# davrempe/humor

Hardware: AMD Instinct MI355X
Metric: fitting closure evaluations/s (stage-3 objective fwd+bwd), batch=32 seq=60 per GPU (higher is better)
Workload: dtype f32

## Files before the change

humor_amd/csrc/rollout.hip:

```cpp
#include <string.h>

#include <algorithm>
#include <list>
#include <unordered_map>
#include <vector>

#include "rollout_persist.h"
#include "rot_math.h"

namespace ha {

constexpr int D_IN = 339, D_STATE = 348, ZD = 48, NJT = 22, NBODY = 21;
template <int ROTW>
struct RawLayout {
  static constexpr int ROOT = 6, RVEL = 6 + ROTW, BODY = 9 + ROTW, JNT = 9 + 22 * ROTW, JVEL = JNT + 66, CONT = JVEL + 66, D = CONT + 9;
};
static_assert(RawLayout<3>::D == 216 && RawLayout<6>::D == 282 && RawLayout<9>::D == 348, "decoder output widths of the three representations");
constexpr int D_INP = 340;
constexpr int SLICE = 64;
constexpr int MAXL = 8;

typedef float f32x16 __attribute__((ext_vector_type(16)));
typedef float vf4 __attribute__((ext_vector_type(4)));

// ... 222 lines not shown
        const vf4 g4 = *reinterpret_cast<const vf4*>(T.gamma + cbase + 32 * hi + 4 * j);
        const vf4 b4 = *reinterpret_cast<const vf4*>(T.beta + cbase + 32 * hi + 4 * j);
        gam[4 * j] = g4.x; gam[4 * j + 1] = g4.y; gam[4 * j + 2] = g4.z; gam[4 * j + 3] = g4.w;
        bet[4 * j] = b4.x; bet[4 * j + 1] = b4.y; bet[4 * j + 2] = b4.z; bet[4 * j + 3] = b4.w;
      }
    }
    float a[32], h[32];
    if (!is_main) load_frag_n<true>(T.skip, 1, L.RT, T.skip_dim, rt, cbase, lane, a);
    else {
      load_frag_n<LEAN>(T.src, T.nsplit_src, L.RT, T.Csrc, rt, cbase, lane, a);
      if (!LEAN && T.mode == 3) load_frag_n(T.hsrc, T.nsplit_h, L.RT, T.Ch, rt, cbase, lane, h);
    }
    HA_TS(1, false);
    HA_TS(2, true);
    if (!LEAN && is_main && T.mode == 1 && T.hsum_dst && tile == 0 && T.nsplit_src > 1) {
      const int c0 = cbase + 32 * hi;
      float* hd = T.hsum_dst + (size_t)rt * T.Csrc * 32 + (size_t)(c0 >> 2) * 128 + (size_t)(lane & 31) * 4;
#pragma unroll
      for (int jq = 0; jq < 8; ++jq)
        if (c0 + 4 * jq < T.Csrc) *reinterpret_cast<vf4*>(hd + (size_t)jq * 128) = vf4{a[4 * jq], a[4 * jq + 1], a[4 * jq + 2], a[4 * jq + 3]};
    }
    if (has_gn) {
      const float inv_n = T.inv_group;
      if (T.mode == 1) {
        if (T.group == SLICE) gn_apply<1>(1, gam, bet, inv_n, a, a);
        else gn_apply<2>(1, gam, bet, inv_n, a, a);
      } else {
        if (T.group == SLICE) gn_apply<1>(3, gam, bet, inv_n, h, a);
        else gn_apply<2>(3, gam, bet, inv_n, h, a);
      }
    }
    HA_TS(3, false);
#pragma unroll
    for (int kp = 0; kp < 32; ++kp) acc = __builtin_amdgcn_mfma_f32_32x32x2f32(a[kp], bw[kp], acc, 0, 0, 0);
  }
#pragma unroll
  for (int i = 0; i < 16; ++i) smem[(wave * 16 + i) * 64 + lane] = acc[i];
  HA_TS(4, true);
  __syncthreads();
  HA_TS(5, false);
  if (threadIdx.x < 256) {
    const int row = threadIdx.x & 31, cq = threadIdx.x >> 5;
    const int reg = (row & 3) + 4 * (row >> 3), half = (row >> 2) & 1;
    vf4 o = {0.f, 0.f, 0.f, 0.f};
#pragma unroll
    for (int w = 0; w < NWT; ++w) o += *reinterpret_cast<const vf4*>(smem + (w * 16 + reg) * 64 + half * 32 + cq * 4);
    const int n = tile * 32 + cq * 4;
    if (ks == 0 && T.bias) {
#pragma unroll
      for (int e = 0; e < 4; ++e)
        if (n + e < T.Nout) o[e] += T.bias[n + e];
    }
    float* dst = T.dst + ((size_t)ks * L.RT + rt) * T.Nout_pad * 32 + (size_t)(n >> 2) * 128 + row * 4;
    *reinterpret_cast<vf4*>(dst) = o;
  }
  HA_TS(6, true);
  HA_TS(7, false);
}

struct FinishLaunch {
  LayerTask t[1];
  float* dst[1];
  int nblk[1];
  int ntasks, RT;
};

__global__ __launch_bounds__(256) void gn_finish_kernel(FinishLaunch F) {
  extern __shared__ __attribute__((aligned(16))) float smem[];
  float (*s_red)[32][8] = reinterpret_cast<float (*)[32][8]>(smem);
  const int b = blockIdx.x, ti = 0;
  const LayerTask& T = F.t[0];
  const int row = threadIdx.x & 31, oct = threadIdx.x >> 5;
  const int slice = b % T.main_slices, rt = b / T.main_slices;
  const int c0 = slice * SLICE + oct * 8;
  const vf4 g0 = *reinterpret_cast<const vf4*>(T.gamma + c0), g1 = *reinterpret_cast<const vf4*>(T.gamma + c0 + 4);
  const vf4 e0 = *reinterpret_cast<const vf4*>(T.beta + c0), e1 = *reinterpret_cast<const vf4*>(T.beta + c0 + 4);
  auto load8 = [&](const float* base, int ns, int C, float (&v)[8]) {
    const size_t stride = (size_t)F.RT * C * 32;
    const float* p = base + (size_t)rt * C * 32 + (size_t)(c0 >> 2) * 128 + (size_t)row * 4;
    vf4 t0[MAXSPLIT], t1[MAXSPLIT];
#pragma unroll
    for (int k = 0; k < MAXSPLIT; ++k) {
      t0[k] = vf4{0.f, 0.f, 0.f, 0.f};
      t1[k] = t0[k];
      if (k < ns) { t0[k] = *reinterpret_cast<const vf4*>(p + k * stride); t1[k] = *reinterpret_cast<const vf4*>(p + k * stride + 128); }
    }
    vf4 a0 = t0[0], a1 = t1[0];
#pragma unroll
    for (int k = 1; k < MAXSPLIT; ++k) { a0 += t0[k]; a1 += t1[k]; }
    v[0] = a0.x; v[1] = a0.y; v[2] = a0.z; v[3] = a0.w; v[4] = a1.x; v[5] = a1.y; v[6] = a1.z; v[7] = a1.w;
  };
  float x[8], da[8];
  if (T.mode == 1) load8(T.src, T.nsplit_src, T.Csrc, x);
  else { load8(T.src, T.nsplit_src, T.Csrc, da); load8(T.hsrc, T.nsplit_h, T.Ch, x); }
  const float gam[8] = {g0.x, g0.y, g0.z, g0.w, g1.x, g1.y, g1.z, g1.w};
  const float bet[8] = {e0.x, e0.y, e0.z, e0.w, e1.x, e1.y, e1.z, e1.w};
  const int per = T.group == SLICE ? 8 : 4, o0 = T.group == SLICE ? 0 : (oct & 4);
  const float inv_n = 1.0f / (float)T.group;
  auto row_sum = [&](int pass, float v) {
    s_red[pass][row][oct] = v;
    __syncthreads();
    float t = 0.f;
    for (int k = 0; k < per; ++k) t += s_red[pass][row][o0 + k];
    return t;
  };
  float p1 = 0.f;
#pragma unroll
  for (int i = 0; i < 8; ++i) p1 += x[i];
  const float mu = row_sum(0, p1) * inv_n;
  float p2 = 0.f;
#pragma unroll
  for (int i = 0; i < 8; ++i) { const float d = x[i] - mu; p2 = fmaf(d, d, p2); }
  const float rstd = rsqrtf(row_sum(1, p2) * inv_n + 1e-5f);
  float out[8];
  if (T.mode == 1) {
#pragma unroll
    for (int i = 0; i < 8; ++i) out[i] = fmaxf((x[i] - mu) * rstd * gam[i] + bet[i], 0.f);
  } else {
    float xh[8], dxh[8], m1 = 0.f, m2 = 0.f;
#pragma unroll
    for (int i = 0; i < 8; ++i) {
      xh[i] = (x[i] - mu) * rstd;
      const float y = xh[i] * gam[i] + bet[i];
      dxh[i] = (y > 0.f ? da[i] : 0.f) * gam[i];
      m1 += dxh[i];
      m2 = fmaf(dxh[i], xh[i], m2);
    }
    m1 = row_sum(2, m1) * inv_n;
    m2 = row_sum(3, m2) * inv_n;
#pragma unroll
    for (int i = 0; i < 8; ++i) out[i] = rstd * (dxh[i] - m1 - xh[i] * m2);
  }
  float* d = F.dst[ti] + (size_t)rt * (T.main_slices * SLICE) * 32 + (size_t)(c0 >> 2) * 128 + (size_t)row * 4;
  *reinterpret_cast<vf4*>(d) = vf4{out[0], out[1], out[2], out[3]};
  *reinterpret_cast<vf4*>(d + 128) = vf4{out[4], out[5], out[6], out[7]};
}


struct GemmTask {
  const float* Wp; const float* bias;
  int ntiles, nslices, Nout;
  const float* src; int Csrc;
  int nrt;
  int epi;
  float slope;
  const float* gamma; const float* beta; int group;
  const float* hsrc; int Ch;
  float* dst_h; float* dst_a; int Cdst;
  int nrg, nwork, per_xcd;
};

constexpr int GEMM_LDS_WAVE = 2 * 8 * 132;

template <int RM, int KS = 1>
__global__ __launch_bounds__(256) void prior_gemm_kernel(GemmTask T) {
  extern __shared__ __attribute__((aligned(16))) float smem[];
  const int wave = threadIdx.x >> 6, lane = threadIdx.x & 63;
  const int w = (int)(blockIdx.x & 7) * T.per_xcd + (int)(blockIdx.x >> 3);
  if ((int)(blockIdx.x >> 3) >= T.per_xcd || w >= T.nwork) return;
  const int cb = w / T.nrg, rg = w % T.nrg;
  const int kpart = KS == 1 ? 0 : wave % KS;
  const int ct0 = KS == 1 ? (cb * 4 + wave) * 2 : (cb * (4 / KS) + wave / KS) * 2;
  const bool tile_ok = ct0 < T.ntiles;
  if (KS == 1 && !tile_ok) return;
  const int ct1 = ct0 + 1 < T.ntiles ? ct0 + 1 : ct0;
  int rt[RM];
#pragma unroll
  for (int m = 0; m < RM; ++m) rt[m] = rg * RM + m < T.nrt ? rg * RM + m : T.nrt - 1;

  f32x16 acc[RM][2];
#pragma unroll
  for (int m = 0; m < RM; ++m)
#pragma unroll
    for (int c = 0; c < 2; ++c)
#pragma unroll
      for (int i = 0; i < 16; ++i) acc[m][c][i] = 0.f;

  const float* wp0 = T.Wp + (size_t)ct0 * T.nslices * 2048 + lane * 4;
  const float* wp1 = T.Wp + (size_t)ct1 * T.nslices * 2048 + lane * 4;
  auto load_b = [&](int slice, float (&b0)[32], float (&b1)[32]) {
#pragma unroll
    for (int j = 0; j < 8; ++j) {
      const vf4 u = *reinterpret_cast<const vf4*>(wp0 + (size_t)slice * 2048 + j * 256);
      const vf4 v = *reinterpret_cast<const vf4*>(wp1 + (size_t)slice * 2048 + j * 256);
      b0[4 * j] = u.x; b0[4 * j + 1] = u.y; b0[4 * j + 2] = u.z; b0[4 * j + 3] = u.w;
      b1[4 * j] = v.x; b1[4 * j + 1] = v.y; b1[4 * j + 2] = v.z; b1[4 * j + 3] = v.w;
    }
  };
  auto load_a = [&](int slice, float (&a)[RM][32]) {
#pragma unroll
    for (int m = 0; m < RM; ++m)
      load_frag<1>(T.src + (size_t)rt[m] * T.Csrc * 32 + (size_t)(slice * 16 + 8 * (lane >> 5)) * 128 + (size_t)(lane & 31) * 4, 0, 8, a[m]);
  };
  auto mma = [&](const float (&a)[RM][32], const float (&b0)[32], const float (&b1)[32]) {
#pragma unroll
    for (int kp = 0; kp < 32; ++kp)
#pragma unroll
      for (int m = 0; m < RM; ++m) {
        acc[m][0] = __builtin_amdgcn_mfma_f32_32x32x2f32(a[m][kp], b0[kp], acc[m][0], 0, 0, 0);
        acc[m][1] = __builtin_amdgcn_mfma_f32_32x32x2f32(a[m][kp], b1[kp], acc[m][1], 0, 0, 0);
      }
  };
  const int nfull_all = T.Csrc / SLICE < T.nslices ? T.Csrc / SLICE : T.nslices;
  const int per_part = (nfull_all + KS - 1) / KS;
  const int sbeg = KS == 1 ? 0 : (kpart * per_part < nfull_all ? kpart * per_part : nfull_all);
  const int nfull = KS == 1 ? nfull_all : ((sbeg + per_part) < nfull_all ? (sbeg + per_part) : nfull_all);
  if (nfull > sbeg && (KS == 1 || tile_ok)) {
    float aA[RM][32], bA0[32], bA1[32], aB[RM][32], bB0[32], bB1[32];
    load_b(sbeg, bA0, bA1);
    load_a(sbeg, aA);
    for (int slice = sbeg; slice < nfull; slice += 2) {
      const int s1 = slice + 1 < nfull ? slice + 1 : slice;
      load_b(s1, bB0, bB1);
      load_a(s1, aB);
      HA_SCHED_FENCE();
      mma(aA, bA0, bA1);
      HA_SCHED_FENCE();
      if (slice + 1 < nfull) {
        const int s2 = slice + 2 < nfull ? slice + 2 : slice + 1;
        load_b(s2, bA0, bA1);
        load_a(s2, aA);
        HA_SCHED_FENCE();
        mma(aB, bB0, bB1);
        HA_SCHED_FENCE();
      }
    }
  }
  if (nfull_all < T.nslices && kpart == KS - 1 && (KS == 1 || tile_ok)) {
    float a[RM][32], b0[32], b1[32];
    load_b(nfull_all, b0, b1);
#pragma unroll
    for (int m = 0; m < RM; ++m) load_frag_n<true>(T.src, 1, 0, T.Csrc, rt[m], nfull_all * SLICE, lane, a[m]);
    mma(a, b0, b1);
  }

  float* sl = smem + wave * GEMM_LDS_WAVE;
  const int row = lane & 31, hh = lane >> 5;
  const int ct = hh ? ct0 + 1 : ct0;
  const bool ct_ok = ct < T.ntiles;
  float gam[32], bet[32];
  if ((T.epi == 1 || T.epi == 3) && ct_ok) {
#pragma unroll
    for (int j = 0; j < 8; ++j) {
      const vf4 g4 = *reinterpret_cast<const vf4*>(T.gamma + ct * 32 + 4 * j);
      const vf4 b4 = *reinterpret_cast<const vf4*>(T.beta + ct * 32 + 4 * j);
      gam[4 * j] = g4.x; gam[4 * j + 1] = g4.y; gam[4 * j + 2] = g4.z; gam[4 * j + 3] = g4.w;
      bet[4 * j] = b4.x; bet[4 * j + 1] = b4.y; bet[4 * j + 2] = b4.z; bet[4 * j + 3] = b4.w;
    }
  } else {
#pragma unroll
    for (int k = 0; k < 32; ++k) { gam[k] = 1.f; bet[k] = 0.f; }
  }
#pragma unroll
  for (int m = 0; m < RM; ++m) {
#pragma unroll
    for (int c = 0; c < 2; ++c)
#pragma unroll
      for (int i = 0; i < 16; ++i) {
        const int r = (i & 3) + 8 * (i >> 2) + 4 * hh, col = lane & 31;
        sl[(c * 8 + (col >> 2)) * 132 + r * 4 + (col & 3)] = acc[m][c][i];
      }
    if (KS == 1) {
      __builtin_amdgcn_fence(__ATOMIC_RELEASE, "wavefront");
      __builtin_amdgcn_wave_barrier();
      __builtin_amdgcn_fence(__ATOMIC_ACQUIRE, "wavefront");
    } else {
      __syncthreads();
    }
    float v[32];
#pragma unroll
    for (int j = 0; j < 8; ++j) {
      vf4 q = *reinterpret_cast<const vf4*>(sl + (hh * 8 + j) * 132 + row * 4);
      if (KS > 1) {
#pragma unroll
        for (int pk = 1; pk < KS; ++pk) q += *reinterpret_cast<const vf4*>(sl + pk * GEMM_LDS_WAVE + (hh * 8 + j) * 132 + row * 4);
      }
      v[4 * j] = q.x; v[4 * j + 1] = q.y; v[4 * j + 2] = q.z; v[4 * j + 3] = q.w;
    }
    if (KS == 1) {
      __builtin_amdgcn_fence(__ATOMIC_RELEASE, "wavefront");
      __builtin_amdgcn_wave_barrier();
      __builtin_amdgcn_fence(__ATOMIC_ACQUIRE, "wavefront");
    } else {
      __syncthreads();
      if (kpart != 0) continue;
    }
    const bool live = ct_ok && rg * RM + m < T.nrt;
    if (T.bias && ct_ok) {
#pragma unroll
      for (int j = 0; j < 8; ++j) {
        const vf4 b4 = *reinterpret_cast<const vf4*>(T.bias + ct * 32 + 4 * j);
        v[4 * j] += b4.x; v[4 * j + 1] += b4.y; v[4 * j + 2] += b4.z; v[4 * j + 3] += b4.w;
      }
    }
    const size_t o = (size_t)rt[m] * T.Cdst * 32 + (size_t)(ct * 8) * 128 + (size_t)row * 4;
    auto store32 = [&](float* base, const float (&x)[32]) {
#pragma unroll
      for (int j = 0; j < 8; ++j) *reinterpret_cast<vf4*>(base + o + (size_t)j * 128) = vf4{x[4 * j], x[4 * j + 1], x[4 * j + 2], x[4 * j + 3]};
    };
    if (T.epi <= 1 && live) store32(T.dst_h, v);
    if (T.epi == 4) {
#pragma unroll
      for (int k = 0; k < 32; ++k) v[k] = v[k] > 0.f ? v[k] : v[k] * T.slope;
      if (live) store32(T.dst_a, v);
    } else if (T.epi == 5) {
      const float* hp = T.hsrc + (size_t)rt[m] * T.Ch * 32 + (size_t)((ct_ok ? ct : ct0) * 8) * 128 + (size_t)row * 4;
#pragma unroll
      for (int j = 0; j < 8; ++j) {
        const vf4 q = *reinterpret_cast<const vf4*>(hp + (size_t)j * 128);
        v[4 * j] *= q.x > 0.f ? 1.f : T.slope; v[4 * j + 1] *= q.y > 0.f ? 1.f : T.slope;
        v[4 * j + 2] *= q.z > 0.f ? 1.f : T.slope; v[4 * j + 3] *= q.w > 0.f ? 1.f : T.slope;
      }
      if (live) store32(T.dst_a, v);
    } else if (T.epi == 1) {
      const float inv_n = 1.0f / (float)T.group;
      if (T.group == SLICE) gn_apply<1>(1, gam, bet, inv_n, v, v);
      else gn_apply<2>(1, gam, bet, inv_n, v, v);
      if (live) store32(T.dst_a, v);
    } else if (T.epi == 3) {
      float h[32];
      const float* hp = T.hsrc + (size_t)rt[m] * T.Ch * 32 + (size_t)((ct_ok ? ct : ct0) * 8) * 128 + (size_t)row * 4;
#pragma unroll
      for (int j = 0; j < 8; ++j) {
        const vf4 q = *reinterpret_cast<const vf4*>(hp + (size_t)j * 128);
        h[4 * j] = q.x; h[4 * j + 1] = q.y; h[4 * j + 2] = q.z; h[4 * j + 3] = q.w;
      }
      const float inv_n = 1.0f / (float)T.group;
      if (T.group == SLICE) gn_apply<1>(3, gam, bet, inv_n, h, v);
      else gn_apply<2>(3, gam, bet, inv_n, h, v);
      if (live) store32(T.dst_a, v);
    }
  }
}

struct GlueParams {
  int B, S, t, RT;
  const float* xT;
  float* xT_next;
  const float* dec_out; int dec_nsplit; int dec_pad;
  const float* pri_out; int pri_nsplit; int pri_pad;
  const float* Gs;
  float* Gs_next;
  const float* t2j;
  float* world;
  float* prior_mu; float* prior_var;
  const float* g_world;
  const float* g_prior_mu; const float* g_prior_var;
  float* g_dec_out;
  float* g_pri_out;
  const float* gx_dir_in;
  float* gx_dir_out;
  const float* gxp_pri; int gxp_pri_nsplit; int gxp_pri_pad;
  const float* gxp_dec; int gxp_dec_nsplit; int gxp_dec_pad;
  float* carry;
  const float* dz_src[MAXL]; int dz_nsplit[MAXL]; int dz_pad[MAXL]; int dz_off[MAXL]; int dz_n;
  float* g_z;
  float* g_past0;
};

__device__ __forceinline__ float tsum(const float* base, int nsplit, int RT, int C, int rt, int c, int row) {
  return base ? slab_sum(base, nsplit, RT, C, rt, c, row) : 0.f;
}

struct PredState {
  float pj[3], jv[3];
  float dB[9], Bin[9], pB[9];
  float ptrans[3], ptvel[3], prvel[3], dR[9], Rin[9], pR[9];
  float raw_aa_b[9], raw_aa_r[9];
};

template <int ROTW>
__device__ __forceinline__ void delta_rot(const float* raw, float R[9]) {
  if constexpr (ROTW == 3) rodrigues(raw, R);
  else if constexpr (ROTW == 6) rot6d_to_rotmat(raw, R);
  else rot9d_to_rotmat(raw, R);
}
template <int ROTW>
__device__ __forceinline__ void delta_rot_bwd(const float* raw, const float gR[9], float* graw) {
  if constexpr (ROTW == 3) rodrigues_bwd(raw, gR, graw);
  else if constexpr (ROTW == 6) rot6d_to_rotmat_bwd(raw, gR, graw);
  else rot9d_to_rotmat_bwd(raw, gR, graw);
}

constexpr int S_X = 0, S_RAW = 352, S_GXN = 704, S_GW = 1056, S_TOTAL = 1408;
constexpr int S_SH = 1408, S_RED = 1424, S_TOTAL_BWD = 1456;

template <int NQ, int NT = 64>
__device__ __forceinline__ void stage_slabs(float* dst, const float* base, int nsplit, int RT, int C, int nch, int rt, int rr,
                                            int lane, bool accumulate) {
  vf4 t[MAXSPLIT][NQ];
#pragma unroll
  for (int sidx = 0; sidx < MAXSPLIT; ++sidx)
#pragma unroll
    for (int i = 0; i < NQ; ++i) t[sidx][i] = vf4{0.f, 0.f, 0.f, 0.f};
  if (base) {
    const size_t stride = (size_t)RT * C * 32;
    const float* p0 = base + (size_t)rt * C * 32 + (size_t)rr * 4;
#pragma unroll
    for (int sidx = 0; sidx < MAXSPLIT; ++sidx)
      if (sidx < nsplit) {
#pragma unroll
        for (int i = 0; i < NQ; ++i) {
          const int q = lane + NT * i;
          if (4 * q < nch) t[sidx][i] = *reinterpret_cast<const vf4*>(p0 + (size_t)sidx * stride + (size_t)q * 128);
        }
      }
  }
#pragma unroll
  for (int i = 0; i < NQ; ++i) {
    vf4 v = {0.f, 0.f, 0.f, 0.f};
#pragma unroll
    for (int sidx = 0; sidx < MAXSPLIT; ++sidx) v += t[sidx][i];
    const int q = lane + NT * i;
#pragma unroll
    for (int e = 0; e < 4; ++e) {
      const int c = 4 * q + e;
      if (c < nch) dst[c] = accumulate ? dst[c] + v[e] : v[e];
    }
  }
}

template <int ROTW, bool DELTA>
__device__ __forceinline__ void predict_joints(const float* sX, const float* sRAW, int j, PredState& s) {
  using RL = RawLayout<ROTW>;
#pragma unroll
  for (int c = 0; c < 3; ++c) {
    s.pj[c] = sRAW[RL::JNT + 3 * j + c] + (DELTA ? sX[207 + 3 * j + c] : 0.f);
    s.jv[c] = sRAW[RL::JVEL + 3 * j + c] + (DELTA ? sX[273 + 3 * j + c] : 0.f);
  }
}
template <int ROTW, bool DELTA>
__device__ __forceinline__ void predict_body(const float* sX, const float* sRAW, int bidx, PredState& s) {
  using RL = RawLayout<ROTW>;
#pragma unroll
  for (int c = 0; c < ROTW; ++c) s.raw_aa_b[c] = sRAW[RL::BODY + ROTW * bidx + c];
  delta_rot<ROTW>(s.raw_aa_b, s.dB);
  if constexpr (DELTA) {
#pragma unroll
// ... 698 lines not shown
      HA_REQUIRE(d->gn_gamma[i] && d->gn_beta[i], "%s: layer %d GroupNorm affine missing", name, i);
      HA_REQUIRE(cin % 16 == 0 && (cin / 16 == 64 || cin / 16 == 32), "%s: hidden width %d needs GroupNorm groups of 32 or 64 channels", name, cin);
    }
    int rc = pack_layer(out[i], d->w[i], d->b[i], d->gn_gamma[i], d->gn_beta[i], cin, d->skip_dim, d->out_dims[i], gn);
    if (rc != HA_OK) return rc;
    cin = d->out_dims[i];
  }
  return HA_OK;
}

struct StashLayout {
  int RT = 0;
  int nsf_pri[MAXL], nsf_dec[MAXL], nsb_dec[MAXL];
  size_t zT = 0, t2j = 0, per_step = 0, steps = 0;
  size_t xT = 0;
  size_t off_G = 0;
  size_t off_dec[MAXL];
  size_t off_hsum[MAXL];
  size_t pri_h[MAXL];
  size_t pri_act[2];
  size_t gx_pri = 0;
  size_t smp_pri[MAXL];
  size_t gx_dir[2], carry = 0, g_dec_out = 0, g_pri_out = 0;
  size_t bwd_dec[MAXL];
  size_t fin[1] = {0};
  bool finish = false;
  bool hsum = false;
  bool single = false;
  bool pipe = false;
  size_t persist_ws = 0;
  size_t off_gn[3] = {0, 0, 0}, off_gl = 0;
  size_t off_ht[3] = {0, 0, 0};
  size_t dz_part = 0;
  int rd_f(int i) const { return single ? 1 : nsf_dec[i]; }
  size_t total = 0;
};

static bool one_launch_fits(int rows) { return g_layer_finish != 2 && (rows <= 32 || (rows <= 256 && g_rollout_pipe != 0)); }

static void make_layout(const ha_humor_net* net, int B, int S, Path path, StashLayout& L) {
  L.RT = ceil_div(B, 32);
  const size_t RT = L.RT;
  for (int i = 0; i < net->n_pri; ++i) L.nsf_pri[i] = ceil_div(net->pri[i].nslices_f, SPB);
  for (int i = 0; i < net->n_dec; ++i) { L.nsf_dec[i] = ceil_div(net->dec[i].nslices_f, SPB); L.nsb_dec[i] = ceil_div(net->dec[i].nslices_b, SPB); }
  L.finish = (L.RT >= 2 && g_layer_finish != 0) || g_layer_finish == 2;
  L.single = path != Path::chain;
  L.pipe = L.single && B > 32;
  L.hsum = !L.finish && !L.single;
  size_t o = 0;
  auto take = [&](size_t n) { size_t r = o; o += (n + 63) / 64 * 64; return r; };
  L.zT = take((size_t)S * RT * ZD * 32);
  L.t2j = take(RT * 32 * 3);
  L.xT = take((size_t)(S + 1) * RT * D_INP * 32);
  size_t p = 0;
  auto ptake = [&](size_t n) { size_t r = p; p += (n + 63) / 64 * 64; return r; };
  L.off_G = ptake(RT * 32 * 12);
  for (int i = 0; i < net->n_dec; ++i) L.off_dec[i] = ptake((size_t)L.rd_f(i) * RT * net->dec[i].Nout_pad * 32);
  for (int i = 0; i + 1 < net->n_dec; ++i) L.off_hsum[i] = L.hsum ? ptake(RT * net->dec[i].Nout_pad * 32) : 0;
  if (L.single) {
    for (int i = 0; i < 3; ++i) L.off_gn[i] = ptake(RT * 16 * 32 * 2);
    L.off_gl = ptake(RT * 32 * 32);
    for (int i = 0; i < 3; ++i) L.off_ht[i] = ptake(RT * 32 * (size_t)net->dec[i].Nout);
  }
  L.per_step = p;
  L.steps = take(p * (size_t)(S + 1));
  size_t widest = 0;
  for (int i = 0; i < net->n_pri; ++i) {
    L.pri_h[i] = take((size_t)S * RT * net->pri[i].Nout_pad * 32);
    if ((size_t)net->pri[i].Nout_pad > widest) widest = net->pri[i].Nout_pad;
    if ((size_t)net->pri[i].Nin_pad > widest) widest = net->pri[i].Nin_pad;
    L.smp_pri[i] = take((size_t)L.nsf_pri[i] * RT * net->pri[i].Nout_pad * 32);
  }
  L.pri_act[0] = take((size_t)S * RT * widest * 32);
  L.pri_act[1] = take((size_t)S * RT * widest * 32);
  L.gx_pri = take((size_t)S * RT * net->pri[0].Nin_pad * 32);
  L.gx_dir[0] = take(RT * D_INP * 32);
  L.gx_dir[1] = take(RT * D_INP * 32);
  L.carry = take(RT * 32 * 16);
  L.g_dec_out = take(RT * net->dec[net->n_dec - 1].Nout_pad * 32);
  L.g_pri_out = take((size_t)S * RT * net->pri[net->n_pri - 1].Nout_pad * 32);
  for (int i = 0; i < net->n_dec; ++i) L.bwd_dec[i] = take((size_t)L.nsb_dec[i] * RT * net->dec[i].Nin_pad * 32);
  if (L.finish)
    L.fin[0] = take(RT * 1280 * 32);
  if (L.single) {
    L.persist_ws = take(L.pipe ? pipe_ws_floats() : persist_ws_floats());
    L.dz_part = take((size_t)S * (L.pipe ? pipe_dz_slots() : persist_dz_slots()) * RT * 32 * ZD);
  }
  L.total = o;
}

static void fwd_task(LayerTask& T, const PackedLayer& L, const float* src, int nsplit_src, const float* skip, float* dst, int nsplit_dst) {
  memset(&T, 0, sizeof(T));
  T.Wp = L.Wf; T.bias = L.bias;
  T.ntiles = L.ntiles_f; T.nslices = L.nslices_f; T.main_slices = L.main_slices; T.Nout = L.Nout; T.Nout_pad = L.Nout_pad;
  T.src = src; T.nsplit_src = nsplit_src; T.Csrc = (L.Cin + 3) & ~3;
  T.skip = skip; T.skip_dim = L.skip;
  T.mode = L.group ? 1 : 0;
  T.gamma = L.gamma; T.beta = L.beta; T.group = L.group ? L.group : 64;
  T.inv_group = 1.0f / (float)T.group;
  T.dst = dst;
  T.spb = SPB; T.nsplit_dst = nsplit_dst;
  T.nblocks = L.ntiles_f * nsplit_dst;
}

static void bwd_task(LayerTask& T, const PackedLayer& L, const float* dsrc, int nsplit_d, int dC, const PackedLayer* Lnext_gn,
                     const float* hsrc, int nsplit_h, float* dst, int nsplit_dst) {
  memset(&T, 0, sizeof(T));
  T.Wp = L.Wb; T.bias = nullptr;
  T.ntiles = L.ntiles_b; T.nslices = L.nslices_b; T.main_slices = L.nslices_b; T.Nout = L.Cin + L.skip; T.Nout_pad = L.Nin_pad;
  T.src = dsrc; T.nsplit_src = nsplit_d; T.Csrc = dC;
  T.mode = Lnext_gn ? 3 : 0;
  if (Lnext_gn) { T.gamma = Lnext_gn->gamma; T.beta = Lnext_gn->beta; T.group = Lnext_gn->group; }
  else T.group = 64;
  T.inv_group = 1.0f / (float)T.group;
  T.hsrc = hsrc; T.nsplit_h = nsplit_h; T.Ch = L.Nout_pad;
  T.dst = dst;
  T.spb = SPB; T.nsplit_dst = nsplit_dst;
  T.nblocks = L.ntiles_b * nsplit_dst;
}

static int launch_layers(LayerLaunch& LL, const StashLayout& L, float* stash, hipStream_t st) {
  if (L.finish) {
    FinishLaunch F;
    memset(&F, 0, sizeof(F));
    F.RT = LL.RT;
    int fb = 0;
    for (int i = 0; i < LL.ntasks; ++i) {
      LayerTask& T = LL.t[i];
      if (T.mode == 0) continue;
      const int k = F.ntasks++;
      F.t[k] = T;
      F.dst[k] = stash + L.fin[i];
      F.nblk[k] = LL.RT * T.main_slices;
      fb += F.nblk[k];
      T.src = F.dst[k]; T.nsplit_src = 1; T.Csrc = T.main_slices * SLICE; T.mode = 0;
      T.hsrc = nullptr; T.nsplit_h = 0;
    }
    if (fb) {
      HA_LAUNCH(gn_finish_kernel, dim3(fb), dim3(256), 4 * 32 * 8 * sizeof(float), st, F);
      HA_LAUNCH_CHECK();
    }
  }
  LayerTask& T0 = LL.t[0];
  const dim3 grid(T0.ntiles, T0.nsplit_dst, LL.RT);
  T0.nblocks *= LL.RT;
  const bool lean = L.finish && T0.mode == 0 && T0.nsplit_src <= 1;
  if (lean) HA_LAUNCH((mlp_layer_kernel<4, true>), grid, dim3(256), 4 * 1024 * sizeof(float), st, LL);
  else HA_LAUNCH((mlp_layer_kernel<4, false>), grid, dim3(256), 4 * 1024 * sizeof(float), st, LL);
  HA_LAUNCH_CHECK();
  return HA_OK;
}


static int launch_prior_gemm(GemmTask& T, hipStream_t st) {
  HA_REQUIRE((T.epi != 1 && T.epi != 3) || (T.ntiles % 2 == 0 && (T.group == 32 || T.group == 64)), "prior GEMM: GroupNorm epilogue needs whole 64-column pairs");
  int ncb = ceil_div(T.ntiles, 8);
  const int rm = g_gemm_rm == 1 || g_gemm_rm == 2 ? g_gemm_rm : ((T.nrt / 2) * ncb >= 2 * 256 ? 2 : 1);
  const int ks = ((g_gemm_ks == 2 || g_gemm_ks == 3) && rm == 1 && T.nslices >= 4 && (g_gemm_ks == 3 || ncb * T.nrt * 4 <= 512)) ? 2 : 1;
  if (ks == 2) ncb = ceil_div(T.ntiles, 4);
  T.nrg = ceil_div(T.nrt, rm);
  T.nwork = ncb * T.nrg;
  T.per_xcd = ceil_div(T.nwork, 8);
  const dim3 grid(T.per_xcd * 8), block(256);
  const size_t lds = 4 * GEMM_LDS_WAVE * sizeof(float);
  if (rm == 2) HA_LAUNCH(prior_gemm_kernel<2>, grid, block, lds, st, T);
  else if (ks == 2) HA_LAUNCH((prior_gemm_kernel<1, 2>), grid, block, lds, st, T);
  else HA_LAUNCH(prior_gemm_kernel<1>, grid, block, lds, st, T);
  HA_LAUNCH_CHECK();
  return HA_OK;
}

static int prior_forward_batched(const ha_humor_net* net, const StashLayout& L, float* stash, int S, hipStream_t st) {
  const int np = net->n_pri;
  for (int l = 0; l < np; ++l) {
    const PackedLayer& P = net->pri[l];
    GemmTask T;
    memset(&T, 0, sizeof(T));
    T.Wp = P.Wf; T.bias = P.bias;
    T.ntiles = P.ntiles_f; T.nslices = P.nslices_f; T.Nout = P.Nout;
    T.src = l == 0 ? stash + L.xT : stash + L.pri_act[(l - 1) & 1];
    T.Csrc = l == 0 ? D_INP : net->pri[l - 1].Nout_pad;
    T.nrt = S * L.RT;
    T.dst_h = stash + L.pri_h[l]; T.Cdst = P.Nout_pad;
    if (l + 1 < np) {
      const PackedLayer& N = net->pri[l + 1];
      T.epi = 1; T.gamma = N.gamma; T.beta = N.beta; T.group = N.group;
      T.dst_a = stash + L.pri_act[l & 1];
    }
    int rc = launch_prior_gemm(T, st);
    if (rc != HA_OK) return rc;
  }
  return HA_OK;
}

static int prior_backward_batched(const ha_humor_net* net, const StashLayout& L, float* stash, int S, hipStream_t st) {
  const int np = net->n_pri;
  for (int l = np - 1; l >= 0; --l) {
    const PackedLayer& P = net->pri[l];
    GemmTask T;
    memset(&T, 0, sizeof(T));
    T.Wp = P.Wb; T.bias = nullptr;
    T.ntiles = P.ntiles_b; T.nslices = P.nslices_b; T.Nout = P.Cin + P.skip;
    T.src = l == np - 1 ? stash + L.g_pri_out : stash + L.pri_act[(l + 1) & 1];
    T.Csrc = P.Nout_pad;
    T.nrt = S * L.RT;
    T.Cdst = P.Nin_pad;
    if (l > 0) {
      T.epi = 3; T.gamma = P.gamma; T.beta = P.beta; T.group = P.group;
      T.hsrc = stash + L.pri_h[l - 1]; T.Ch = net->pri[l - 1].Nout_pad;
      T.dst_a = stash + L.pri_act[l & 1];
    } else {
      T.epi = 0; T.dst_h = stash + L.gx_pri;
    }
    int rc = launch_prior_gemm(T, st);
    if (rc != HA_OK) return rc;
  }
  return HA_OK;
}

constexpr int MAX_GROUPS = 8;

static void group_plan(int B, bool piped, int& ngroups, int& rows_per_group) {
  if (piped) {
    rows_per_group = 256;
    ngroups = ceil_div(B, 256);
    return;
  }
  const int RT = ceil_div(B, 32);
  int n = g_rollout_groups > 0 ? g_rollout_groups : (RT == 2 ? 2 : 1);
  if (n > MAX_GROUPS) n = MAX_GROUPS;
  if (n > RT) n = RT;
  rows_per_group = ceil_div(RT, n) * 32;
  ngroups = ceil_div(B, rows_per_group);
}

static int layout_knobs() { return (g_layer_finish & 3) | ((g_rollout_pipe & 1) << 2) | ((g_rollout_groups & 0xff) << 3); }

static size_t group_stash_floats(const ha_humor_net* net, int rows, int S, bool may_one_launch) {
  StashLayout L;
  make_layout(net, rows, S, Path::chain, L);
  size_t best = L.total;
  if (may_one_launch && one_launch_fits(rows)) {
    make_layout(net, rows, S, Path::one_launch, L);
    best = std::max(best, L.total);
  }
  return best;
}

static CallPlan rollout_plan(const ha_humor_net* net, int B, int S) {
  CallPlan p;
  if (g_rollout_persist != 0 && persist_usable(net->persist) && one_launch_fits(std::min(B, 256))) {
    p.piped = B > 32;
    const bool lean = g_rollout_persist_bwd != 0 && (!p.piped || g_rollout_pipe_bwd != 0);
    p.path = lean ? Path::one_launch_lean : Path::one_launch;
  }
  group_plan(B, p.piped, p.ngroups, p.rows_per_group);
  p.group_floats = p.ngroups > 1 ? group_stash_floats(net, p.rows_per_group, S, p.piped) : 0;
  return p;
}

static bool adjoint_one_launch(const CallPlan& p, int rows) {
  if (p.path == Path::one_launch_lean) return true;
  return p.path == Path::one_launch && g_rollout_persist_bwd != 0 && (rows <= 32 || g_rollout_pipe_bwd != 0);
}

}

using namespace ha;

extern "C" int ha_humor_net_create(ha_humor_net** out, int device, const ha_mlp_desc* decoder, const ha_mlp_desc* prior) {
  HA_REQUIRE(out && decoder && prior, "ha_humor_net_create: null argument");
  const int raw = decoder->out_dims[decoder->n_linear - 1];
  const int rotw = raw == RawLayout<3>::D ? 3 : raw == RawLayout<6>::D ? 6 : raw == RawLayout<9>::D ? 9 : 0;
  HA_REQUIRE(decoder->in_dim == D_IN + ZD && decoder->skip_dim == ZD && rotw != 0,
             "ha_humor_net_create: decoder must map [339+48] -> 216 / 282 / 348 (out_rot_rep aa / 6d / 9d) with a 48-d latent skip "
             "(got in=%d skip=%d out=%d)", decoder->in_dim, decoder->skip_dim, raw);
  HA_REQUIRE(prior->in_dim == D_IN && prior->skip_dim == 0 && prior->out_dims[prior->n_linear - 1] == 2 * ZD,
             "ha_humor_net_create: prior must map 339 -> 96");
  HA_REQUIRE(prior->n_linear <= 2 * decoder->n_linear, "ha_humor_net_create: the prior may be at most twice as deep as the decoder");
  DeviceGuard guard(device);
  HA_REQUIRE(guard.ok, "ha_humor_net_create: cannot select device %d", device);
  ha_humor_net* net = new ha_humor_net();
  net->device = device;
  net->n_dec = decoder->n_linear;
  net->n_pri = prior->n_linear;
  net->rotw = rotw;
  int rc;
  if ((rc = pack_mlp(net->dec, decoder, "decoder")) != HA_OK || (rc = pack_mlp(net->pri, prior, "prior")) != HA_OK ||
      (rc = persist_create(&net->persist, device, decoder)) != HA_OK) {
    ha_humor_net_destroy(net);
    return rc;
  }
  *out = net;
  return HA_OK;
}

extern "C" int ha_humor_net_destroy(ha_humor_net* net) {
  if (!net) return HA_OK;
  DeviceGuard guard(net->device);
  persist_destroy(net->persist);
  net->persist = nullptr;
  for (PackedLayer* arr : {net->dec, net->pri})
    for (int i = 0; i < MAXL; ++i) {
      void* ptrs[] = {arr[i].Wf, arr[i].Wb, arr[i].bias, arr[i].gamma, arr[i].beta};
      for (void* p : ptrs)
        if (p) (void)hipFree(p);
    }
  delete net;
  return HA_OK;
}

extern "C" int ha_humor_persist_status(const ha_humor_net* net, int* available, unsigned int* error_word, int64_t* launches) {
  HA_REQUIRE(net && available && error_word && launches, "ha_humor_persist_status: null argument");
  *error_word = persist_error_word(net->persist);
  *launches = persist_launches(net->persist) + (persist_launches_bwd(net->persist) << 32);
  *available = persist_usable(net->persist) ? 1 : 0;
  return HA_OK;
}

extern "C" int ha_humor_persist_ack(const ha_humor_net* net) {
// ... 693 lines not shown
```

Before: 612.8.

## Add cost-model planner choosing column-tile width and K-split depth for prior GEMM

Generalizes the prior GEMM kernel with a TN template parameter so one wave can own a single 32-column tile, and allows a four-way K split in addition to two. A small cost model picks tile width and split depth by estimated waves per SIMD times the serial MFMA chain. The aim is more parallelism and a shorter critical path when the layer has few tiles. The epilogue sync is also reworked so non-leader K-parts return early. The planner only runs when the ks knob is 2 or 3, so the default path may not change.

New measurement: 627.8 (median of 6 runs). +2.4%, better.

```diff
diff --git a/humor_amd/csrc/rollout.hip b/humor_amd/csrc/rollout.hip
--- a/humor_amd/csrc/rollout.hip
+++ b/humor_amd/csrc/rollout.hip
@@ -398,27 +398,29 @@
 
 constexpr int GEMM_LDS_WAVE = 2 * 8 * 132;
 
-template <int RM, int KS = 1>
+template <int RM, int KS = 1, int TN = 2>
 __global__ __launch_bounds__(256) void prior_gemm_kernel(GemmTask T) {
+  static_assert(KS == 1 || RM == 1, "the K split is built for one row tile per wave");
+  static_assert((KS == 1 || KS == 2 || KS == 4) && (TN == 1 || TN == 2), "prior_gemm_kernel: unsupported shape");
   extern __shared__ __attribute__((aligned(16))) float smem[];
   const int wave = threadIdx.x >> 6, lane = threadIdx.x & 63;
   const int w = (int)(blockIdx.x & 7) * T.per_xcd + (int)(blockIdx.x >> 3);
   if ((int)(blockIdx.x >> 3) >= T.per_xcd || w >= T.nwork) return;
   const int cb = w / T.nrg, rg = w % T.nrg;
   const int kpart = KS == 1 ? 0 : wave % KS;
-  const int ct0 = KS == 1 ? (cb * 4 + wave) * 2 : (cb * (4 / KS) + wave / KS) * 2;
+  const int ct0 = KS == 1 ? (cb * 4 + wave) * TN : (cb * (4 / KS) + wave / KS) * TN;
   const bool tile_ok = ct0 < T.ntiles;
   if (KS == 1 && !tile_ok) return;
-  const int ct1 = ct0 + 1 < T.ntiles ? ct0 + 1 : ct0;
+  const int ct1 = TN == 2 && ct0 + 1 < T.ntiles ? ct0 + 1 : ct0;
   int rt[RM];
 #pragma unroll
   for (int m = 0; m < RM; ++m) rt[m] = rg * RM + m < T.nrt ? rg * RM + m : T.nrt - 1;
 
-  f32x16 acc[RM][2];
+  f32x16 acc[RM][TN];
 #pragma unroll
   for (int m = 0; m < RM; ++m)
 #pragma unroll
-    for (int c = 0; c < 2; ++c)
+    for (int c = 0; c < TN; ++c)
 #pragma unroll
       for (int i = 0; i < 16; ++i) acc[m][c][i] = 0.f;
 
@@ -428,9 +430,11 @@
 #pragma unroll
     for (int j = 0; j < 8; ++j) {
       const vf4 u = *reinterpret_cast<const vf4*>(wp0 + (size_t)slice * 2048 + j * 256);
-      const vf4 v = *reinterpret_cast<const vf4*>(wp1 + (size_t)slice * 2048 + j * 256);
       b0[4 * j] = u.x; b0[4 * j + 1] = u.y; b0[4 * j + 2] = u.z; b0[4 * j + 3] = u.w;
-      b1[4 * j] = v.x; b1[4 * j + 1] = v.y; b1[4 * j + 2] = v.z; b1[4 * j + 3] = v.w;
+      if (TN == 2) {
+        const vf4 v = *reinterpret_cast<const vf4*>(wp1 + (size_t)slice * 2048 + j * 256);
+        b1[4 * j] = v.x; b1[4 * j + 1] = v.y; b1[4 * j + 2] = v.z; b1[4 * j + 3] = v.w;
+      }
     }
   };
   auto load_a = [&](int slice, float (&a)[RM][32]) {
@@ -444,7 +448,7 @@
 #pragma unroll
       for (int m = 0; m < RM; ++m) {
         acc[m][0] = __builtin_amdgcn_mfma_f32_32x32x2f32(a[m][kp], b0[kp], acc[m][0], 0, 0, 0);
-        acc[m][1] = __builtin_amdgcn_mfma_f32_32x32x2f32(a[m][kp], b1[kp], acc[m][1], 0, 0, 0);
+        if (TN == 2) acc[m][TN - 1] = __builtin_amdgcn_mfma_f32_32x32x2f32(a[m][kp], b1[kp], acc[m][TN - 1], 0, 0, 0);
       }
   };
   const int nfull_all = T.Csrc / SLICE < T.nslices ? T.Csrc / SLICE : T.nslices;
@@ -483,7 +487,8 @@
   float* sl = smem + wave * GEMM_LDS_WAVE;
   const int row = lane & 31, hh = lane >> 5;
   const int ct = hh ? ct0 + 1 : ct0;
-  const bool ct_ok = ct < T.ntiles;
+  const bool ct_ok = hh < TN && ct < T.ntiles;
+  const int hs = hh < TN ? hh : 0;
   float gam[32], bet[32];
   if ((T.epi == 1 || T.epi == 3) && ct_ok) {
 #pragma unroll
@@ -500,7 +505,7 @@
 #pragma unroll
   for (int m = 0; m < RM; ++m) {
 #pragma unroll
-    for (int c = 0; c < 2; ++c)
+    for (int c = 0; c < TN; ++c)
 #pragma unroll
       for (int i = 0; i < 16; ++i) {
         const int r = (i & 3) + 8 * (i >> 2) + 4 * hh, col = lane & 31;
@@ -512,14 +517,15 @@
       __builtin_amdgcn_fence(__ATOMIC_ACQUIRE, "wavefront");
     } else {
       __syncthreads();
+      if (kpart != 0) return;
     }
     float v[32];
 #pragma unroll
     for (int j = 0; j < 8; ++j) {
-      vf4 q = *reinterpret_cast<const vf4*>(sl + (hh * 8 + j) * 132 + row * 4);
+      vf4 q = *reinterpret_cast<const vf4*>(sl + (hs * 8 + j) * 132 + row * 4);
       if (KS > 1) {
 #pragma unroll
-        for (int pk = 1; pk < KS; ++pk) q += *reinterpret_cast<const vf4*>(sl + pk * GEMM_LDS_WAVE + (hh * 8 + j) * 132 + row * 4);
+        for (int pk = 1; pk < KS; ++pk) q += *reinterpret_cast<const vf4*>(sl + pk * GEMM_LDS_WAVE + (hs * 8 + j) * 132 + row * 4);
       }
       v[4 * j] = q.x; v[4 * j + 1] = q.y; v[4 * j + 2] = q.z; v[4 * j + 3] = q.w;
     }
@@ -527,9 +533,6 @@
       __builtin_amdgcn_fence(__ATOMIC_RELEASE, "wavefront");
       __builtin_amdgcn_wave_barrier();
       __builtin_amdgcn_fence(__ATOMIC_ACQUIRE, "wavefront");
-    } else {
-      __syncthreads();
-      if (kpart != 0) continue;
     }
     const bool live = ct_ok && rg * RM + m < T.nrt;
     if (T.bias && ct_ok) {
@@ -1534,20 +1537,53 @@
 }
 
 
+struct GemmPlan { int rm, tn, ks, ncb; };
+
+static GemmPlan plan_prior_gemm(int ntiles, int nslices, int nrt, int epi, int rm_knob, int ks_knob) {
+  GemmPlan P;
+  P.ncb = ceil_div(ntiles, 8);
+  P.rm = rm_knob == 1 || rm_knob == 2 ? rm_knob : ((nrt / 2) * P.ncb >= 2 * 256 ? 2 : 1);
+  P.tn = 2;
+  P.ks = 1;
+  const bool split_on = ks_knob == 2 || ks_knob == 3;
+  if (!split_on || P.rm == 2) return P;
+  const bool force = ks_knob == 3;
+  if (!force && P.ncb * nrt * 4 > 512) return P;
+  const bool gn = epi == 1 || epi == 3;
+  constexpr int SIMDS = 1024;
+  int best = ceil_div(ceil_div(ntiles, 2) * nrt, SIMDS) * nslices * 2;
+  if (force) best = nslices * 2;
+  for (int tn = 2; tn >= (gn ? 2 : 1); --tn)
+    for (int ks = 1; ks <= 4; ks *= 2) {
+      if (ks > 1 && nslices < 2 * ks) continue;
+      const int waves = ceil_div(ntiles, tn) * nrt * ks;
+      if (!force && waves > 2 * SIMDS) continue;
+      const int chain = ceil_div(nslices, ks) * tn;
+      const int cost = force ? chain : ceil_div(waves, SIMDS) * chain;
+      if (cost < best || (force && cost == best && ks > P.ks)) { best = cost; P.tn = tn; P.ks = ks; P.ncb = ceil_div(ntiles, tn * 4 / ks); }
+    }
+  return P;
+}
+
 static int launch_prior_gemm(GemmTask& T, hipStream_t st) {
   HA_REQUIRE((T.epi != 1 && T.epi != 3) || (T.ntiles % 2 == 0 && (T.group == 32 || T.group == 64)), "prior GEMM: GroupNorm epilogue needs whole 64-column pairs");
-  int ncb = ceil_div(T.ntiles, 8);
-  const int rm = g_gemm_rm == 1 || g_gemm_rm == 2 ? g_gemm_rm : ((T.nrt / 2) * ncb >= 2 * 256 ? 2 : 1);
-  const int ks = ((g_gemm_ks == 2 || g_gemm_ks == 3) && rm == 1 && T.nslices >= 4 && (g_gemm_ks == 3 || ncb * T.nrt * 4 <= 512)) ? 2 : 1;
-  if (ks == 2) ncb = ceil_div(T.ntiles, 4);
-  T.nrg = ceil_div(T.nrt, rm);
-  T.nwork = ncb * T.nrg;
+  const GemmPlan P = plan_prior_gemm(T.ntiles, T.nslices, T.nrt, T.epi, g_gemm_rm, g_gemm_ks);
+  T.nrg = ceil_div(T.nrt, P.rm);
+  T.nwork = P.ncb * T.nrg;
   T.per_xcd = ceil_div(T.nwork, 8);
   const dim3 grid(T.per_xcd * 8), block(256);
   const size_t lds = 4 * GEMM_LDS_WAVE * sizeof(float);
-  if (rm == 2) HA_LAUNCH(prior_gemm_kernel<2>, grid, block, lds, st, T);
-  else if (ks == 2) HA_LAUNCH((prior_gemm_kernel<1, 2>), grid, block, lds, st, T);
-  else HA_LAUNCH(prior_gemm_kernel<1>, grid, block, lds, st, T);
+  const int shape = P.rm * 100 + P.ks * 10 + P.tn;
+  switch (shape) {
+    case 212: HA_LAUNCH(prior_gemm_kernel<2>, grid, block, lds, st, T); break;
+    case 112: HA_LAUNCH(prior_gemm_kernel<1>, grid, block, lds, st, T); break;
+    case 122: HA_LAUNCH((prior_gemm_kernel<1, 2>), grid, block, lds, st, T); break;
+    case 142: HA_LAUNCH((prior_gemm_kernel<1, 4>), grid, block, lds, st, T); break;
+    case 111: HA_LAUNCH((prior_gemm_kernel<1, 1, 1>), grid, block, lds, st, T); break;
+    case 121: HA_LAUNCH((prior_gemm_kernel<1, 2, 1>), grid, block, lds, st, T); break;
+    case 141: HA_LAUNCH((prior_gemm_kernel<1, 4, 1>), grid, block, lds, st, T); break;
+    default: HA_REQUIRE(false, "prior GEMM: no kernel for RM %d KS %d TN %d", P.rm, P.ks, P.tn);
+  }
   HA_LAUNCH_CHECK();
   return HA_OK;
 }
```
